# snayfach/MicrobeCensus

Hardware: AMD Instinct MI355X
Metric: reads/sec searched vs marker DB + AGS abs-error, 150 bp @ 1/2/4/8 GPU (higher is better)
Workload: dtype u8/int32

## Files before the change

### include/mcensus.h

```cpp
#ifndef MCENSUS_H
#define MCENSUS_H
#include <stdint.h>
#ifdef __cplusplus
extern "C" {
#endif

typedef struct mc_handle mc_handle;

typedef struct mc_row {
    int32_t query, subject;
    double ident;
    int32_t alnlen, mismatch, gapopen, qstart, qend, sstart, send;
    double loge, bits;
    int32_t score, nmatch;
} mc_row;

typedef struct mc_best_hit {
    int32_t read, family, aln, target_len;
    double bits;
} mc_best_hit;

typedef struct mc_stats {
    int64_t reads, seed_tasks, gap_tasks, hsps, rows, reads_with_rows, classified;
    int64_t bucket_lookups, key_probes;
// ... 34 lines not shown
int mc_search_classes(mc_handle *h, const uint8_t *rows, int64_t nreads, int32_t stride, int64_t first_read_id);
int64_t mc_result_best_classes(mc_handle *h, const uint8_t **cls);
int mc_result_class_reads(mc_handle *h, int64_t *out );
int64_t mc_debug_classes_prologue(mc_handle *h, const uint8_t *rows, int64_t nreads, int32_t stride, uint32_t *perm, uint32_t *start, int64_t *word0,
                                  uint8_t *sorted, int64_t sorted_cap, float *ms);

int mc_upload(mc_handle *h, const uint8_t *reads, int64_t nreads);
int mc_attach(mc_handle *h, const void *device_reads, int64_t nreads);
int mc_run(mc_handle *h, int64_t first_read_id);
int mc_run_range(mc_handle *h, int64_t first, int64_t count, int64_t first_read_id);

int mc_range_begin(mc_handle *h, int64_t first, int64_t count, int64_t first_read_id);
int mc_range_end(mc_handle *h);
int mc_ranges_in_flight(const mc_handle *h);
int64_t mc_ranges_translated_ahead(const mc_handle *h);

int64_t mc_debug_stage(mc_handle *h, int what, void *dst, int64_t cap_bytes, int32_t *record_bytes);
void mc_debug_live(int64_t out[4]);

int mc_set_counting(mc_handle *h, int on);

int64_t mc_result_rows(mc_handle *h, const mc_row **rows);
int64_t mc_result_best_hits(mc_handle *h, const mc_best_hit **hits);
int mc_result_stats(mc_handle *h, mc_stats *out);

int mc_write_m8(mc_handle *h, const char *path, int append);
int mc_write_m8_named(mc_handle *h, const char *path, int append, const char *const *query_names, int64_t n_names, int64_t first_read_id);

int mc_grid_classify(mc_handle *h, const double *aln_covs, int32_t n_cov, const int32_t *max_pids, int32_t n_pid, const double *min_scores, int32_t n_score,
                     int64_t *count_hits, int64_t *count_aln, double *count_cov);
// ... 111 lines not shown
```

### microbecensus_amd/_native.py

```python
import ctypes as C
import gzip
import json
import math
import os
import sys

import numpy as np

_HERE = os.path.dirname(os.path.abspath(__file__))
LIB_PATH = os.path.join(_HERE, "libmcensus_hip.so")
DATA_DIR = os.path.join(_HERE, "data")


class McRow(C.Structure):
    _fields_ = [("query", C.c_int32), ("subject", C.c_int32), ("ident", C.c_double), ("alnlen", C.c_int32),
                ("mismatch", C.c_int32), ("gapopen", C.c_int32), ("qstart", C.c_int32), ("qend", C.c_int32),
                ("sstart", C.c_int32), ("send", C.c_int32), ("loge", C.c_double), ("bits", C.c_double),
                ("score", C.c_int32), ("nmatch", C.c_int32)]


class McBestHit(C.Structure):
    _fields_ = [("read", C.c_int32), ("family", C.c_int32), ("aln", C.c_int32), ("target_len", C.c_int32),
                ("bits", C.c_double)]

# ... 66 lines not shown
    lib.mc_set_run.argtypes = [C.c_void_p, C.c_int32, C.c_double, C.POINTER(C.c_double), C.POINTER(C.c_double), C.POINTER(C.c_int32), C.POINTER(C.c_int32)]
    lib.mc_search.argtypes = [C.c_void_p, C.c_void_p, C.c_int64, C.c_int64]
    lib.mc_search_varlen.argtypes = [C.c_void_p, C.c_void_p, C.c_void_p, C.c_int64, C.c_int64]
    lib.mc_upload.argtypes = [C.c_void_p, C.c_void_p, C.c_int64]
    lib.mc_run.argtypes = [C.c_void_p, C.c_int64]
    lib.mc_attach.argtypes = [C.c_void_p, C.c_void_p, C.c_int64]
    lib.mc_run_range.argtypes = [C.c_void_p, C.c_int64, C.c_int64, C.c_int64]
    lib.mc_set_counting.argtypes = [C.c_void_p, C.c_int]
    lib.mc_debug_stage.restype = C.c_int64
    lib.mc_debug_stage.argtypes = [C.c_void_p, C.c_int, C.c_void_p, C.c_int64, C.POINTER(C.c_int32)]
    lib.mc_range_begin.argtypes = [C.c_void_p, C.c_int64, C.c_int64, C.c_int64]
    lib.mc_range_end.argtypes = [C.c_void_p]
    lib.mc_ranges_in_flight.argtypes = [C.c_void_p]
    lib.mc_ranges_translated_ahead.restype = C.c_int64
    lib.mc_ranges_translated_ahead.argtypes = [C.c_void_p]
    lib.mc_result_rows.restype = C.c_int64
    lib.mc_result_rows.argtypes = [C.c_void_p, C.POINTER(C.POINTER(McRow))]
    lib.mc_result_best_hits.restype = C.c_int64
    lib.mc_result_best_hits.argtypes = [C.c_void_p, C.POINTER(C.POINTER(McBestHit))]
    lib.mc_result_stats.argtypes = [C.c_void_p, C.POINTER(McStats)]
    lib.mc_write_m8.argtypes = [C.c_void_p, C.c_char_p, C.c_int]
    lib.mc_write_m8_named.argtypes = [C.c_void_p, C.c_char_p, C.c_int, C.POINTER(C.c_char_p), C.c_int64, C.c_int64]
    lib.mc_reader_last_error.restype = C.c_char_p
    lib.mc_set_host_threads.restype = None
    lib.mc_set_host_threads.argtypes = [C.c_int32]
    lib.mc_reader_open.restype = C.c_void_p
    lib.mc_reader_open.argtypes = [C.POINTER(C.c_char_p), C.c_int32, C.c_int32, C.c_int64, C.c_int32, C.c_int32, C.c_double, C.c_double, C.c_double, C.c_int32, C.c_char_p]
    lib.mc_reader_open_range.restype = C.c_void_p
    lib.mc_reader_open_range.argtypes = [C.c_char_p, C.c_int64, C.c_int64, C.c_int32, C.c_int64, C.c_int32, C.c_int32, C.c_double, C.c_double, C.c_double]
    lib.mc_reader_run.restype = C.c_int64
# ... 95 lines not shown
    lib.mc_coverage_depth.argtypes = [C.c_void_p, C.c_void_p, C.c_int64]
    lib.mc_coverage_ms.restype = C.c_float
    lib.mc_coverage_ms.argtypes = [C.c_void_p]
    lib.mc_set_ties.argtypes = [C.c_void_p, C.c_int, C.c_void_p, C.c_int32]
    lib.mc_ties_read.argtypes = [C.c_void_p, C.c_void_p, C.c_void_p, C.c_void_p, C.c_void_p, C.POINTER(C.c_int64), C.POINTER(C.c_int64)]
    lib.mc_ties_coverage_read.argtypes = [C.c_void_p, C.c_void_p, C.c_void_p, C.c_void_p]
    lib.mc_ties_ms.restype = C.c_float
    lib.mc_ties_ms.argtypes = [C.c_void_p]
    lib.mc_debug_live.restype = None
    lib.mc_debug_live.argtypes = [C.POINTER(C.c_int64)]
    _lib = lib
    return lib


EXPORTED_SYMBOLS = ["mc_last_error", "mc_device_count", "mc_open", "mc_close", "mc_set_index_cache", "mc_index_cache_check", "mc_open_rapdb", "mc_marker_count", "mc_marker_name", "mc_set_families", "mc_rapdb_verify", "mc_rapdb_write", "mc_index_view", "mc_set_run", "mc_search", "mc_search_varlen",
                    "mc_upload", "mc_attach", "mc_run", "mc_run_range", "mc_set_counting", "mc_debug_stage", "mc_range_begin", "mc_range_end", "mc_ranges_in_flight", "mc_ranges_translated_ahead", "mc_result_rows", "mc_result_best_hits", "mc_result_stats", "mc_write_m8", "mc_write_m8_named",
                    "mc_reader_last_error", "mc_set_host_threads", "mc_reader_open", "mc_reader_open_range", "mc_reader_open_bz2_part", "mc_bz2_blocks", "mc_gz_chunks", "mc_reader_open_gz_part", "mc_reader_gz_provide", "mc_reader_gz_end_state", "mc_reader_gz_finish", "mc_reader_run", "mc_reader_reads", "mc_reader_get_stats", "mc_reader_times", "mc_reader_describe", "mc_dupset_open", "mc_dupset_close", "mc_dupset_walk", "mc_reader_take", "mc_reader_close", "mc_reader_trim", "mc_count_bases", "mc_quality_offset",
                    "mc_reader_start", "mc_reader_fetch", "mc_reader_join", "mc_reader_read_len", "mc_reader_nreads", "mc_search_files", "mc_search_files_multi", "mc_set_keep_rows", "mc_set_best_hits_only", "mc_grid_classify", "mc_bootstrap", "mc_bootstrap_ms",
                    "mc_fit_weights", "mc_weights_mue", "mc_fit_weights_ms",
                    "mc_genome_open", "mc_genome_close", "mc_genome_set_library", "mc_simulate", "mc_train_library", "mc_train_times",
                    "mc_genome_set_read_lengths", "mc_simulate_varlen", "mc_train_library_bases",
                    "mc_community_open", "mc_community_close", "mc_community_set_library", "mc_community_simulate", "mc_community_library", "mc_community_member_reads",
                    "mc_community_times",
                    "mc_set_run_classes", "mc_search_classes", "mc_result_best_classes", "mc_result_class_reads", "mc_debug_classes_prologue", "mc_reader_open_classes", "mc_reader_stride",
                    "mc_set_abundance", "mc_abundance_reset", "mc_abundance_read", "mc_abundance_ms",
                    "mc_set_coverage", "mc_coverage_read", "mc_coverage_depth", "mc_coverage_ms",
                    "mc_set_ties", "mc_ties_read", "mc_ties_coverage_read", "mc_ties_ms", "mc_debug_live"]


class DupSet:

# ... 652 lines not shown
    def set_counting(self, on):
        self._check(self.lib.mc_set_counting(self.h, 1 if on else 0), "mc_set_counting")

    def range_begin(self, first, count, first_read_id=0):
        self._check(self.lib.mc_range_begin(self.h, first, count, first_read_id), "mc_range_begin")

    def range_end(self):
        self._check(self.lib.mc_range_end(self.h), "mc_range_end")

    def ranges_in_flight(self):
        return self.lib.mc_ranges_in_flight(self.h)

    def ranges_translated_ahead(self):
        return int(self.lib.mc_ranges_translated_ahead(self.h))

    def run_range(self, first, count, first_read_id=0):
        self._check(self.lib.mc_run_range(self.h, first, count, first_read_id), "mc_run_range")

    def debug_stage(self, what):
        rec = C.c_int32(0)
        n = self.lib.mc_debug_stage(self.h, what, None, 0, C.byref(rec))
        if n < 0:
            raise RuntimeError("mc_debug_stage failed: %s" % self.lib.mc_last_error().decode())
        buf = np.zeros(n, np.uint8)
        if n and self.lib.mc_debug_stage(self.h, what, buf.ctypes.data_as(C.c_void_p), n, C.byref(rec)) != n:
            raise RuntimeError("mc_debug_stage failed: %s" % self.lib.mc_last_error().decode())
        return buf.reshape(-1, rec.value) if rec.value else buf

    def gap_counts(self):
        v = self.debug_stage(4).reshape(-1).view("<u4")
# ... 142 lines not shown
```

### microbecensus_amd/csrc/mc_ahead.h

```cpp
#pragma once
#include <stdint.h>
#include <algorithm>

struct McAheadKey { uint64_t reads_gen; int64_t first, count; int32_t read_len, FP; uint64_t tables_gen; };
struct McAhead { McAheadKey key = {0, 0, 0, 0, 0, 0}; bool live = false; };

inline int64_t mc_ahead_predict(int64_t first, int64_t count, int64_t nreads, int64_t *next_first)
{
    *next_first = 0;
    if (first < 0 || count <= 0 || first > nreads - count) return 0;
    const int64_t at = first + count;
    const int64_t n = std::min(count, nreads - at);
    if (n <= 0) return 0;
    *next_first = at;
    return n;
}

inline void mc_ahead_offer(McAhead &a, const McAheadKey &k) { a.key = k; a.live = true; }

inline void mc_ahead_drop(McAhead &a) { a.live = false; }

inline int64_t mc_ahead_take(McAhead &a, const McAheadKey &want)
{
    const bool was = a.live;
    a.live = false;
    const McAheadKey &k = a.key;
    if (!was || want.count <= 0 || k.count <= 0 || k.reads_gen != want.reads_gen || k.first != want.first || k.read_len != want.read_len || k.FP != want.FP || k.tables_gen != want.tables_gen) return 0;
    return std::min(k.count, want.count);
}
```

### microbecensus_amd/csrc/mc_hip.hip

```cpp
#include "mc_hip_common.h"
#include "k_translate_seg.h"
#include "k_enumerate.h"
#include "k_eval_seeds.h"
#include "k_gapped.h"
#include "k_order.h"
#include "k_finish.h"
#include "k_grid.h"
#include "k_simulate.h"
#include "k_community.h"
#include "k_varlen.h"
#include "k_classes.h"
#include "k_bootstrap.h"
#include "k_wfit.h"
#include "mc_pieces.h"
#include "mc_ahead.h"
#include "mc_owned.h"
#include "mc_abund.h"

#include <map>

struct McCtx {
    McStream stream; hipStream_t side = nullptr, side2 = nullptr;
    McEvent ev[8], ev_fork, ev_join, ev_join2;
    int64_t cap_reads = 0; int pool_len = 0;
    int ts_staged = -1;
    uint32_t cap_tasks = 0, cap_gaps = 0, cap_hsps = 0, cap_rows = 0;
    McDev<uint8_t> d_frames_base; uint8_t *d_frames = nullptr;
    McDev<unsigned long long> d_stats;
    McDev<McSeedTask> d_tasks; McDev<McGapTask> d_gaps; McDev<McHsp> d_hsps, d_v, d_tmp;
    McDev<uint64_t> d_k64, d_hkeys, d_hplace, d_places; McDev<uint32_t> d_idx, d_idxo, d_heads, d_scan, d_gsz, d_nv, d_ghist;
    McDev<uint32_t> d_counters;
    McDev<McRow> d_rows; McDev<uint32_t> d_nrow, d_rowoff; McDev<McBestHit> d_best, d_bestof; McDev<uint8_t> d_low, d_cand;
    McDev<McGapCell> d_gws_full; McDev<uint32_t> d_retry, d_retry2; int gap_threads_full = 0;
    McDev<unsigned long long> d_gtab; uint32_t gtab_slots = 0; McDev<uint32_t> d_gleader; McDev<McFlankOut> d_fout;
    McPin<uint32_t> h_c; McPin<unsigned long long> h_stats; McPin<McBestHit> h_best; size_t h_best_cap = 0;
    const uint8_t *reads = nullptr; int64_t n = 0, first_read_id = 0, first = 0;
    int ahead_from = -1;
    bool own_a0 = true;
    uint32_t ntasks = 0, ngaps = 0, gpad = 0, nh = 0, nh_all = 0, nheads = 0, nrows = 0, nbest = 0, nsegs = 0;
    bool busy = false;
};

struct mc_handle {
    McHostIndex H;
    std::vector<int32_t> fam;
    int nfam = 0, device = 0;
    McDev<uint8_t> d_res_base; uint8_t *d_res = nullptr; McDev<uint32_t> d_off, d_bstart, d_post; McDev<unsigned long long> d_post8; McDev<uint16_t> d_keys; McDev<int32_t> d_fam;
    McDev<McTables> d_T; McDev<McClassPars> d_P;
    McTables hT; McClassPars hP;
    int read_len = 0, FP = 0; bool run_set = false;
    McDev<uint32_t> d_bitmap;
    McDev<McBucketRec> d_rec;
// ... 5 lines not shown
    bool best_only = false;
    bool rows_stay = false;
    float train_ms[3] = {0, 0, 0};
    float comm_ms[2] = {0, 0};
    int64_t train_bases = 0;
    float boot_ms = 0;
    float wfit_ms = 0;
    McAbundance ab;
    McPin<uint8_t> stage_pin[2]; McDev<uint8_t> stage_dev[2]; size_t stage_bytes = 0; McStream copy_stream;
    int64_t nreads = 0, cap_own = 0;
    McDev<uint8_t> d_reads;
    const uint8_t *reads_dev = nullptr;
    McCtx ctx;
    McStream ahead_stream; McEvent ahead_ev[2][2]; int ahead_p = 0; bool ahead_wait = false;
    McAhead ahead; uint64_t reads_gen = 0, tables_gen = 0; int64_t ahead_used = 0;
    McPin<mc_row> pin_slot[2]; size_t pin_slot_cap[2] = {0, 0}; int pin_cur = 0;
    McStream side, side2;
    McStream rows_stream; McEvent ev_rows; bool rows_pending = false, rows_ever = false;
    std::vector<mc_row> all_rows, split_rows;
    const mc_row *res_rows = nullptr; int64_t n_res_rows = 0;
    std::vector<mc_best_hit> best; mc_stats stats;
    McCtx *best_from = nullptr; uint32_t best_count = 0;
    std::map<int, McTables> vl_tables; double vl_thr = 0;
    McClasses cls = {}; bool cls_set = false, cls_results = false; std::vector<McClassPars> cls_pars;
    std::vector<uint8_t> best_cls; int64_t cls_reads[MC_CL_BINS] = {};
};

static void ahead_drop(mc_handle *h)
{
    if (h->ahead_wait) { (void)hipStreamSynchronize(h->ahead_stream); h->ahead_wait = false; }
// ... 56 lines not shown
static int open_impl(mc_handle *h, const int32_t *marker_family, int32_t nfam, int32_t device)
{
    int ndev = 0;
    double t0 = mc_now();
    if (hipGetDeviceCount(&ndev) != hipSuccess || ndev <= 0) { g_err = "no HIP device available: libmcensus_hip has no CPU fallback"; return -1; }
    if (device < 0 || device >= ndev) { g_err = "device index out of range"; return -1; }
    if (nfam > 32) { g_err = "at most 32 gene families are supported"; return -1; }
    const int nseq = h->H.nseq;
    if (nseq > 32767) { g_err = "more than 32767 markers: the HSP sort key (read<<43 | subject<<28 | hit order) holds 15 bits of subject index"; return -1; }
    for (int s = 0; s < nseq; s++) if ((int)(h->H.off[s + 1] - h->H.off[s]) > MC_GAP_W - 8) { g_err = "marker longer than the gapped-extension workspace"; return -1; }
    if (marker_family) h->fam.assign(marker_family, marker_family + nseq); else h->fam.assign((size_t)nseq, 0);
    h->nfam = nfam; h->device = device;
    HIPCK(hipSetDevice(device));
    HIPCK(hipFree(nullptr));
    MC_OT("  HIP runtime, device", t0);
    if (h->side.create() || h->side2.create()) return -1;
    {
        McCtx &c = h->ctx;
        if (c.stream.create()) return -1;
        c.side = h->side; c.side2 = h->side2;
        for (auto &e : c.ev) if (e.create()) return -1;
        if (c.ev_fork.create(false) || c.ev_join.create(false) || c.ev_join2.create(false)) return -1;
        if (c.d_counters.alloc(C_N) || c.d_stats.alloc(S_N) || c.d_ghist.alloc((size_t)MC_GS_BINS)) return -1;
        if (c.h_c.alloc(C_N) || c.h_stats.alloc(S_N)) return -1;
    }
    if (h->rows_stream.create() || h->ev_rows.create(false)) return -1;
    if (h->ahead_stream.create()) return -1;
    for (auto &pair : h->ahead_ev) for (auto &e : pair) if (e.create()) return -1;
    const McHostIndex &H = h->H;
    if (H.res.size() >= MC_TASK_ABS_LIMIT) { g_err = "marker database too large: more than 16 M residues (MC_TASK_W3)"; return -1; }
    if (h->d_res_base.alloc(H.res.size() + 128) || h->d_off.alloc(H.off.size()) || h->d_bstart.alloc(H.bstart.size()) || h->d_post.alloc(H.post.size() + 1) || h->d_post8.alloc((H.post.size() + 1) * MC_POST_WORDS) ||
        h->d_keys.alloc(H.keys.size()) || h->d_fam.alloc((size_t)nseq) || h->d_T.alloc(1) || h->d_P.alloc(1)) return -1;
    HIPCK(hipMemset(h->d_res_base, MC_INV, H.res.size() + 128));
    h->d_res = h->d_res_base + 64;
    h->ab.bind(nseq, (size_t)H.nres, h->d_off);
    if (h->d_bitmap.alloc(H.bitmap.size()) || h->d_filt.alloc(H.filt.size()) || h->d_wild.alloc(H.wild.size()) || h->d_pair.alloc(H.pair.size()) || h->d_rt.alloc(H.rt.size())) return -1;
    if (!H.rec.empty() && h->d_rec.alloc(H.rec.size())) return -1;
    {
        McUploader up;
        if (up.init() || up.put(h->d_res, H.res.data(), H.res.size()) || up.put(h->d_off, H.off.data(), H.off.size() * 4) || up.put(h->d_bstart, H.bstart.data(), H.bstart.size() * 4) ||
            up.put(h->d_post, H.post.data(), H.post.size() * 4) || up.put(h->d_keys, H.keys.data(), H.keys.size() * 2) || up.put(h->d_fam, h->fam.data(), (size_t)nseq * 4) ||
            up.put(h->d_bitmap, H.bitmap.data(), H.bitmap.size() * 4) || up.put(h->d_pair, H.pair.data(), H.pair.size() * 4) || up.put(h->d_wild, H.wild.data(), H.wild.size() * 4) ||
// ... 176 lines not shown
{
    if (nreads <= c.cap_reads && h->read_len <= c.pool_len) return 0;
    if (h->best_from == &c) best_materialize(h);
    ahead_drop(h);
    double t0 = mc_now();
    int64_t cap = nreads;
    if (cap > (1 << 21) - 1) { g_err = "batch larger than 2097151 reads"; return -1; }
    const int64_t L = h->read_len;
    c.cap_reads = 0;
    c.cap_tasks = (uint32_t)std::min<int64_t>(cap * (L + 32) + (1 << 20) + (int64_t)256 * 32 * MC_EN_BLK, 0x7fffffff);
    const int64_t ev_pad = (int64_t)256 * 8 * (MC_EV_BS / 64) * MC_EV_BLK;
    c.cap_gaps = (uint32_t)std::min<int64_t>(cap * (L / 8 + 8) + (1 << 18) + ev_pad, (1 << 27) - 2);
    c.cap_hsps = (uint32_t)std::min<int64_t>(cap * (L / 3 + 8) + (1 << 20) + ev_pad, 0x7fffffff);
    c.cap_rows = (uint32_t)std::min<int64_t>(cap * 16 + (1 << 20), 0x7fffffff);
    c.gap_threads_full = 16 * 1024;
    if (c.d_frames_base.alloc((size_t)cap * 6 * h->FP + 128) || c.d_tasks.alloc(c.cap_tasks) ||
        c.d_gaps.alloc(c.cap_gaps) || c.d_hsps.alloc(c.cap_hsps) || c.d_v.alloc(c.cap_hsps) ||
        c.d_tmp.alloc((size_t)c.cap_hsps * 2) || c.d_k64.alloc(c.cap_hsps) || c.d_hkeys.alloc(c.cap_hsps) || c.d_hplace.alloc(c.cap_hsps) || c.d_places.alloc(c.cap_hsps) || c.d_idx.alloc(c.cap_hsps) ||
        c.d_idxo.alloc(c.cap_hsps) || c.d_heads.alloc((size_t)cap + 2) || c.d_scan.alloc((size_t)4100) || c.d_gsz.alloc(c.cap_hsps) || c.d_nv.alloc((size_t)cap + 1) || c.d_rows.alloc(c.cap_rows) ||
        c.d_low.alloc((size_t)cap + 64) || c.d_cand.alloc((size_t)cap + 64) || c.d_nrow.alloc((size_t)cap + 1) || c.d_rowoff.alloc((size_t)cap + 1) || c.d_best.alloc((size_t)cap + 1) || c.d_bestof.alloc((size_t)cap + 1) ||
        c.d_gws_full.alloc((size_t)c.gap_threads_full * MC_GAP_W) || c.d_retry.alloc((size_t)c.cap_gaps * 2 + (size_t)cap + 1) || c.d_retry2.alloc((size_t)c.cap_gaps * 2) || c.d_gleader.alloc((size_t)c.cap_gaps) ||
        c.d_fout.alloc((size_t)c.cap_gaps * 2))
        return -1;
    c.d_frames = c.d_frames_base + 64;
    HIPCK(hipMemsetAsync(c.d_frames_base, MC_INV, 64, c.stream));
    if (c.h_best.alloc((size_t)cap + 1)) return -1;
    c.h_best_cap = (size_t)cap + 1;
    c.cap_reads = cap; c.pool_len = (int)L;
    HIPCK(hipStreamSynchronize(c.stream));
    MC_OT("ensure_capacity (pools)", t0);
    return 0;
}

static int reads_reserve(mc_handle *h, int64_t nreads)
{
    const int64_t need = nreads * (int64_t)h->read_len + 16;
    if (need > h->cap_own) { reads_change(h); if (h->d_reads.alloc((size_t)need)) return -1; h->cap_own = need; }
    return 0;
}

// ... 70 lines not shown
            fprintf(stderr, "fh-worst read: %llu stacked HSPs, %.3f Mcycles:", w[0] & 0xFFFFF, (double)(w[0] >> 20) / 1e6);
            for (int k = 0; k < 8; k++) fprintf(stderr, " %s %.3f", nm[k], (double)w[1 + k] / 1e6);
            fprintf(stderr, "\n");
            unsigned long long z12[12] = {0, 0, 0, 0, 0, 0, 0, 0, 0, 0, 0, 0};
            HIPCK(hipMemcpyToSymbol(HIP_SYMBOL(g_fh_worst), z12, sizeof z12));
        }
        unsigned long long z[8] = {0, 0, 0, 0, 0, 0, 0, 0};
        HIPCK(hipMemcpyToSymbol(HIP_SYMBOL(g_fh_acc), z, sizeof z)); HIPCK(hipMemcpyToSymbol(HIP_SYMBOL(g_fh_cnt), z, sizeof z));
    }
    return 0;
}
#else
static int exp_timing_dump(mc_handle *, McCtx &, char) { return 0; }
#endif

static int stage_a0(mc_handle *h, McCtx &c, hipStream_t st, const uint8_t *reads, int64_t at, int64_t n, hipEvent_t e0, hipEvent_t e1)
{
    const int L = h->read_len, FP = h->FP;
    uint8_t *frames = c.d_frames + at * 6 * FP;
    HIPCK(hipEventRecord(e0, st));
    const size_t lds_rest = (size_t)MC_TS_NLNF(FP) * 8 + (size_t)MC_TS_THREADS * MC_TS_STRIDE(FP);
    const size_t lds_staged = (size_t)MC_TS_STAGE(L) + lds_rest, lds_direct = (size_t)MC_TS_STAGE(0) + lds_rest;
    static const int ts_force = getenv("MC_TS_STAGED") ? atoi(getenv("MC_TS_STAGED")) : -1;
    const size_t cu_lds = 160 * 1024 - 1024;
    const bool staged = ts_force >= 0 ? ts_force != 0 : cu_lds / lds_staged >= cu_lds / lds_direct;
    const size_t lds = staged ? lds_staged : lds_direct;
    c.ts_staged = staged ? 1 : 0;
    const unsigned ts_blocks = (unsigned)((n + MC_TS_READS - 1) / MC_TS_READS);
    if (staged) {
        if (lds > 48 * 1024) HIPCK(hipFuncSetAttribute((const void *)k_translate_seg<true>, hipFuncAttributeMaxDynamicSharedMemorySize, (int)lds));
        k_translate_seg<true><<<dim3(ts_blocks), dim3(MC_TS_THREADS), lds, st>>>(h->d_T, reads, L, n, frames, FP, h->d_segtab);
    } else {
        if (lds > 48 * 1024) HIPCK(hipFuncSetAttribute((const void *)k_translate_seg<false>, hipFuncAttributeMaxDynamicSharedMemorySize, (int)lds));
        k_translate_seg<false><<<dim3(ts_blocks), dim3(MC_TS_THREADS), lds, st>>>(h->d_T, reads, L, n, frames, FP, h->d_segtab);
// ... 3 lines not shown
}

static int stage_a(mc_handle *h, McCtx &c, int64_t covered)
{
    const int64_t n = c.n;
    const int L = h->read_len, FP = h->FP;
    hipStream_t st = c.stream;
    McIndex X = dev_index(h);
    c.ntasks = c.ngaps = c.gpad = c.nh = c.nheads = c.nrows = c.nbest = c.nsegs = 0;
    HIPCK(hipMemsetAsync(c.d_counters, 0, sizeof(uint32_t) * C_N, st));
    HIPCK(hipMemsetAsync(c.d_stats, 0, sizeof(unsigned long long) * S_N, st));
    if (h->best_only) HIPCK(hipMemsetAsync(c.d_cand, 0, (size_t)n, st));
    HIPCK(hipMemsetAsync(c.d_low, 0, (size_t)n, st));
    c.own_a0 = covered < n;
    if (!c.own_a0) HIPCK(hipEventRecord(c.ev[1], st));
    else if (stage_a0(h, c, st, c.reads + covered * L, covered, n - covered, c.ev[0], c.ev[1])) return -1;
    if (exp_timing_dump(h, c, 'a')) return -1;
    const int64_t threads = n * 6;
    if (h->fast_enum) {
        const bool enq = !h->count_traffic;
        const size_t per_wave = enq ? MC_ENQ_WAVE_LDS(FP, L) : sizeof(McEnWave) + MC_EN_WAVE_LDS(FP, L);
        int waves = 0, bpc = 1;
        {
            static const int shapes_q[][2] = {{8, 2}, {4, 4}, {16, 1}, {12, 1}, {4, 3}, {8, 1}, {4, 2}, {4, 1}};
            static const int shapes_c[][2] = {{12, 2}, {8, 3}, {4, 6}, {4, 5}, {16, 1}, {8, 2}, {4, 4}, {12, 1}, {4, 3}, {8, 1}, {4, 2}, {4, 1}};
            if (enq) { for (const auto &sh : shapes_q) if (!waves && (size_t)sh[1] * (64 + sh[0] * per_wave) <= 160 * 1024) { waves = sh[0]; bpc = sh[1]; } }
            else for (const auto &sh : shapes_c) if (!waves && (size_t)sh[1] * (64 + sh[0] * per_wave) <= 160 * 1024) { waves = sh[0]; bpc = sh[1]; }
        }
        if (!waves) { g_err = "reads too long for the seed kernel's LDS layout"; return -1; }
        const size_t lds2 = 64 + waves * per_wave;
#define MC_LAUNCH_EN(KERNEL, WV)                                                                                                                   \
// ... 193 lines not shown
    McResults R(true, &h->split_rows);
    R.tot.range_splits = 1;
    int64_t off = 0, step = std::max<int64_t>(1, count / 2);
    while (off < count) {
        const int64_t nb = std::min<int64_t>(step, count - off);
        rc = run_range_once(h, first + off, nb, first_read_id + off);
        if (rc == -2 && nb > 1) { step = std::max<int64_t>(1, nb / 2); R.tot.range_splits++; continue; }
        if (rc) return rc;
        R.take(h);
        off += nb;
    }
    h->res_rows = R.rows.data(); h->n_res_rows = (int64_t)R.rows.size(); h->best.swap(R.best); h->best_from = nullptr; h->stats = R.tot;
    return 0;
}

static int range_begin(mc_handle *h, McCtx &c, int64_t first, int64_t count, int64_t first_read_id)
{
    if (ensure_capacity(h, c, count)) return -1;
    c.reads = h->reads_dev + first * h->read_len; c.n = count; c.first_read_id = first_read_id; c.first = first;
    const int64_t covered = mc_ahead_take(h->ahead, ahead_key(h, first, count));
    if (h->ahead_wait) { HIPCK(hipStreamWaitEvent(c.stream, h->ahead_ev[h->ahead_p][1], 0)); h->ahead_wait = false; }
    c.ahead_from = covered ? h->ahead_p : -1;
    if (covered) { h->ahead_used++; h->ahead_p ^= 1; }
    const int rc = stage_a(h, c, covered);
    if (rc) { (void)hipStreamSynchronize(c.stream); return rc; }
    c.busy = true;
    return 0;
}

static int ahead_issue(mc_handle *h, McCtx &c, int64_t first, int64_t count)
{
    if (count <= 0 || count > c.cap_reads || h->read_len > c.pool_len || first < 0 || first + count > h->nreads || !h->reads_dev) return 0;
    ahead_drop(h);
    HIPCK(hipStreamWaitEvent(h->ahead_stream, c.ev[4], 0));
    h->ahead_wait = true;
    if (stage_a0(h, c, h->ahead_stream, h->reads_dev + first * h->read_len, 0, count, h->ahead_ev[h->ahead_p][0], h->ahead_ev[h->ahead_p][1])) { ahead_drop(h); return -1; }
    mc_ahead_offer(h->ahead, ahead_key(h, first, count));
    return 0;
}

static void best_materialize(mc_handle *h)
{
    McCtx *c = h->best_from;
    if (!c) return;
    h->best_from = nullptr;
    const uint32_t nb = h->best_count;
    std::sort(c->h_best.get(), c->h_best + nb, [](const McBestHit &x, const McBestHit &y) { return x.read < y.read; });
    h->best.resize(nb);
    for (uint32_t i = 0; i < nb; i++) { const McBestHit &x = c->h_best[i]; mc_best_hit &o = h->best[i]; o.read = x.read; o.family = x.family; o.aln = x.aln; o.target_len = x.target_len; o.bits = x.bits; }
}

static int range_end(mc_handle *h, McCtx &c, int64_t next_first = 0, int64_t next_count = 0)
{
    c.busy = false;
    h->cls_results = false;
    memset(&h->stats, 0, sizeof h->stats);
    h->res_rows = nullptr; h->n_res_rows = 0; h->best.clear(); h->best_from = nullptr;
    h->stats.reads = c.n;
    int rc = stage_wait(c);
    if (rc == 0) rc = stage_b(h, c);
    if (rc == 0 && MC_AHEAD_ON) rc = ahead_issue(h, c, next_first, next_count);
    if (rc == 0 && (rc = stage_wait(c)) == 0 && (rc = stage_c(h, c)) == 0) rc = stage_d(h, c);
    if (rc == 0) rc = stage_wait(c);
    if (rc == 0 && c.h_c[C_OVERFLOW]) { g_err = "row buffer overflow"; rc = -2; }
    if (rc) { (void)hipStreamSynchronize(c.stream); ahead_drop(h); return rc; }
    h->pin_cur ^= 1;
    c.nrows = (c.nh && !h->best_only) ? c.h_c[C_ROWS] : 0u; c.nsegs = c.h_c[C_SEGS]; c.nbest = c.h_c[C_BEST];
    const bool abund = h->ab.active() && !h->best_only;
    if (abund && h->ab.launch(c.d_rows, std::min(c.nrows, c.cap_rows), c.stream)) return -1;
    if ((size_t)c.nrows > h->pin_slot_cap[h->pin_cur] && !rows_stay(h)) {
        (void)hipStreamSynchronize(h->rows_stream);
        const size_t want = (size_t)c.nrows + c.nrows / 4 + 1024;
        McPin<mc_row> nb, ob;
        if (nb.alloc(want)) { g_err = "out of pinned host memory for the rows"; return -1; }
        h->pin_slot[h->pin_cur] = std::move(nb); h->pin_slot_cap[h->pin_cur] = want;
        const int other = h->pin_cur ^ 1;
        if (h->pin_slot_cap[other] < want && ob.alloc(want) == 0) { h->pin_slot[other] = std::move(ob); h->pin_slot_cap[other] = want; }
    }
    rc = stage_e(h, c);
    if (rc) { (void)hipStreamSynchronize(c.stream); (void)hipStreamSynchronize(h->rows_stream); return rc; }
    if (c.nrows && !rows_stay(h)) { HIPCK(hipEventRecord(h->ev_rows, h->rows_stream)); h->rows_pending = true; h->rows_ever = true; }
    if ((rc = stage_wait(c)) != 0) return rc;
    if (abund) h->ab.range_done(c.n);
    h->res_rows = rows_stay(h) ? nullptr : (const mc_row *)h->pin_slot[h->pin_cur]; h->n_res_rows = rows_stay(h) ? 0 : (int64_t)c.nrows;
    h->best_from = &c; h->best_count = c.nbest;
#ifdef MC_EXP_TIMING
    { const char *nm[6] = {"staging/other", "append", "lookup", "push", "setup", "expand"}; for (int k = 0; k < 6; k++) fprintf(stderr, "timing %-14s %8.3f Mcycles/wave-avg  %10llu entries\n", nm[k], (double)c.h_stats[4 + k] / 4096.0 / 1e6, c.h_stats[10 + k]); }
#endif
    h->stats.bucket_lookups += (int64_t)c.h_stats[S_LOOKUPS]; h->stats.key_probes += (int64_t)c.h_stats[S_KEYPROBES]; h->stats.seed_tasks += (int64_t)c.h_stats[S_TASKS];
    h->stats.seed_exact_asks += (int64_t)c.h_stats[S_EXACT]; h->stats.seed_wild_asks += (int64_t)c.h_stats[S_WILD]; h->stats.seed_pair_asks += (int64_t)c.h_stats[S_PAIRS]; h->stats.seed_probes += (int64_t)c.h_stats[S_PROBES];
    h->stats.gap_tasks += c.ngaps - c.gpad; h->stats.hsps += c.nh_all; h->stats.rows += c.nrows; h->stats.reads_with_rows += c.nsegs;
    const float ms_tr = (c.own_a0 ? ev_ms(c.ev[0], c.ev[1]) : 0.0f) + (c.ahead_from >= 0 ? ev_ms(h->ahead_ev[c.ahead_from][0], h->ahead_ev[c.ahead_from][1]) : 0.0f);
    h->stats.ms_translate += ms_tr; h->stats.ms_seed += ev_ms(c.ev[1], c.ev[2]); h->stats.ms_eval += ev_ms(c.ev[2], c.ev[3]);
    h->stats.ms_gapped += ev_ms(c.ev[3], c.ev[4]); h->stats.ms_sort += ev_ms(c.ev[4], c.ev[5]); h->stats.ms_finish += ev_ms(c.ev[5], c.ev[6]); h->stats.ms_total += ms_tr + ev_ms(c.ev[1], c.ev[6]);
    h->stats.classified = (int64_t)c.nbest;
    return 0;
}

static int range_check(mc_handle *h, int64_t first, int64_t count)
{
    if (!h || !h->run_set) { g_err = "mc_set_run() must be called first"; return -1; }
    if (first < 0 || count < 0 || first + count > h->nreads) { g_err = "range outside the resident read set"; return -1; }
    if (count > (1 << 21) - 1) { g_err = "batch larger than 2097151 reads"; return -1; }
    HIPCK(hipSetDevice(h->device));
    return 0;
}

static int run_range_once(mc_handle *h, int64_t first, int64_t count, int64_t first_read_id)
{
    if (range_check(h, first, count)) return -1;
    if (count == 0) { memset(&h->stats, 0, sizeof h->stats); h->res_rows = nullptr; h->n_res_rows = 0; h->best.clear(); h->best_from = nullptr; return 0; }
    McCtx &c = h->ctx;
    const int rc = range_begin(h, c, first, count, first_read_id);
    if (rc) return rc;
    return range_end(h, c);
}

extern "C" int mc_range_begin(mc_handle *h, int64_t first, int64_t count, int64_t first_read_id)
{
    if (range_check(h, first, count)) return -1;
    if (count <= 0) { g_err = "mc_range_begin: an empty range"; return -1; }
    if (h->pipe_nout) { g_err = "mc_range_begin: a range is in flight already (mc_range_end first)"; return -1; }
    const int rc = range_begin(h, h->ctx, first, count, first_read_id);
    if (rc) return rc;
    h->pipe_nout = 1;
    return 0;
}

static int range_end_next(mc_handle *h, int64_t first, int64_t count, bool predict)
{
    if (predict) count = mc_ahead_predict(h->ctx.first, h->ctx.n, h->nreads, &first);
    return range_end(h, h->ctx, first, count);
}

extern "C" int64_t mc_ranges_translated_ahead(const mc_handle *h) { return h ? h->ahead_used : 0; }

extern "C" int mc_range_end(mc_handle *h)
{
    if (!h) { g_err = "null handle"; return -1; }
    if (h->pipe_nout == 0) { g_err = "mc_range_end: no range in flight"; return -1; }
    HIPCK(hipSetDevice(h->device));
    h->pipe_nout = 0;
    return range_end_next(h, 0, 0, true);
}

extern "C" int mc_ranges_in_flight(const mc_handle *h) { return h ? h->pipe_nout : 0; }

extern "C" int64_t mc_debug_stage(mc_handle *h, int what, void *dst, int64_t cap_bytes, int32_t *record_bytes)
{
    if (!h || !h->run_set || what < 0 || what > 5) { g_err = "mc_debug_stage: bad argument"; return -1; }
    if (h->pipe_nout) { g_err = "mc_debug_stage: ranges are in flight"; return -1; }
    HIPCK(hipSetDevice(h->device));
    ahead_drop(h);
    const McCtx &c = h->ctx;
    if (what == 4) {
        if (!c.h_c) { g_err = "mc_debug_stage: no range has run"; return -1; }
        const uint32_t v[3] = {c.h_c[C_ITEMS], c.h_c[C_RETRY], c.h_c[C_RETRY2]};
        if (record_bytes) *record_bytes = (int32_t)sizeof(uint32_t);
// ... 79 lines not shown
            cv.notify_all();
            if (rc <= 0) return;
        }
    });
    h->all_rows.clear();
    if (h->keep_rows && expect_reads > 0) h->all_rows.reserve((size_t)expect_reads * 2 + 1024);
    McResults R(h->keep_rows, &h->all_rows);
    const uint8_t *saved_reads = h->reads_dev; const int64_t saved_n = h->nreads;
    bool pending = false;
    auto collect = [&]() { if (pending) { pending = false; R.take(h); } };
    auto release = [&](int k) { std::unique_lock<std::mutex> lk(mu); slot[k].state = 0; cv.notify_all(); };
    auto reads_at = [&](int k) { reads_change(h); h->reads_dev = slot[k].dev; h->nreads = slot[k].n; };
    auto end_batch = [&](int k, int next) -> int {
        if (next >= 0) reads_at(next);
        h->pipe_nout = 0;
        int r = range_end_next(h, 0, next >= 0 ? slot[next].n : 0, false);
        if (r == -2) { reads_at(k); r = mc_run_range(h, 0, slot[k].n, first_read_id + slot[k].first); if (next >= 0) reads_at(next); }
        if (r) return r;
        pending = true;
        release(k);
        return 0;
    };
    int rc = 0, flying = -1;
    for (int k = 0;; k ^= 1) {
        {
            bool ready;
            { std::unique_lock<std::mutex> lk(mu); ready = slot[k].state != 0; }
            if (!ready && flying >= 0) { if ((rc = end_batch(flying, -1)) != 0) break; flying = -1; collect(); }
        }
        { std::unique_lock<std::mutex> lk(mu); cv.wait(lk, [&] { return slot[k].state != 0; }); }
        if (slot[k].state == 2) { if (slot[k].rc < 0) { rc = (int)slot[k].rc; if (!up_err.empty()) g_err = up_err; } break; }
        if (flying >= 0) { if ((rc = end_batch(flying, k)) != 0) break; flying = -1; }
        else reads_at(k);
        if ((rc = mc_range_begin(h, 0, slot[k].n, first_read_id + slot[k].first)) != 0) break;
        flying = k;
        collect();
    }
    if (rc == 0 && flying >= 0) { rc = end_batch(flying, -1); flying = -1; }
    if (rc == 0) collect();
    if (h->pipe_nout) { h->pipe_nout = 0; (void)range_end(h, h->ctx); }
    ahead_drop(h);
    { std::unique_lock<std::mutex> lk(mu); abort_up = true; cv.notify_all(); }
    uploader.join();
    reads_change(h);
    h->reads_dev = saved_reads; h->nreads = saved_n;
    if (rc) return rc;
    h->res_rows = R.rows.data(); h->n_res_rows = (int64_t)R.rows.size(); h->best.swap(R.best); h->best_from = nullptr; h->stats = R.tot;
    return 0;
}
// ... 103 lines not shown
        if (e == hipSuccess && pars) e = hipMemcpy(h->d_P, &h->hP, sizeof(McClassPars), hipMemcpyHostToDevice);
        if (rc == 0 && e != hipSuccess) { g_err = std::string("restoring the run's tables: ") + hipGetErrorString(e); rc = -1; }
        return rc;
    }
};

template <class BlockOf> static int run_pieces(mc_handle *h, McLenBorrow &len, const std::vector<McPiece> &pieces, BlockOf block_of, const McClassPars *pars, McResults &R)
{
    auto same_bin = [](const McPiece &a, const McPiece &b) { return a.tag == b.tag && a.L == b.L && a.bin_first == b.bin_first && a.bin_n == b.bin_n; };
    auto begin = [&](const McPiece &q, const McPiece *before) -> int {
        if (!before || !same_bin(*before, q)) {
            if (len.use(q.L, pars ? pars + q.tag : nullptr)) return -1;
            reads_change(h);
            h->reads_dev = block_of(q); h->nreads = q.bin_n;
        }
        return mc_range_begin(h, q.first, q.n, q.bin_first + q.first);
    };
    int rc = pieces.empty() ? 0 : begin(pieces[0], nullptr);
    for (size_t j = 0; rc == 0 && j < pieces.size(); j++) {
        const McPiece &q = pieces[j];
        const McPiece *nx = j + 1 < pieces.size() ? &pieces[j + 1] : nullptr;
        const bool ahead = nx && same_bin(q, *nx);
        h->pipe_nout = 0;
        rc = range_end_next(h, ahead ? nx->first : 0, ahead ? nx->n : 0, false);
        if (rc == -2) rc = mc_run_range(h, q.first, q.n, q.bin_first + q.first);
        if (rc) break;
        if (nx && (rc = begin(*nx, &q)) != 0) break;
        R.take(h, q.tag);
    }
    if (h->pipe_nout) { h->pipe_nout = 0; (void)range_end(h, h->ctx); }
    ahead_drop(h);
    return rc;
}


static int vl_bucket(McDevBuf &B, hipStream_t st, const uint8_t *d_bases, const int64_t *d_off, int64_t nreads, int64_t total, uint8_t **d_sorted,
                     uint32_t **d_perm, std::vector<uint32_t> &start, std::vector<int64_t> &boff)
{
    const uint32_t ntiles = (uint32_t)((nreads + MC_VL_TILE - 1) / MC_VL_TILE);
// ... 919 lines not shown
}

extern "C" int mc_simulate(mc_genome *g, int32_t read_len, int64_t first, int64_t n, uint64_t seed, uint64_t library_id, uint8_t *dst_host)
{
    if (!g || first < 0 || n < 0 || (n > 0 && !dst_host)) { g_err = "mc_simulate: bad argument"; return -1; }
    if (simulate_begin(g, read_len)) return -1;
    if (n == 0) return 0;
    return simulate_to_host(g, read_len, first, n, sim_key(seed, library_id), dst_host, "mc_simulate");
}

static int train_range(mc_handle *h, int64_t first, int64_t count, int64_t first_read_id, const McGridPars &G, unsigned long long *d_bins, size_t nbins,
                       hipEvent_t e0, hipEvent_t e1, mc_stats &tot)
{
    if (count <= 0) return 0;
    McCtx &c = h->ctx;
    int rc = range_begin(h, c, first, count, first_read_id);
    if (rc == 0) rc = range_end(h, c);
    if (rc == -2 && count > 1) {
        tot.range_splits++;
        const int64_t a = count / 2;
        if ((rc = train_range(h, first, a, first_read_id, G, d_bins, nbins, e0, e1, tot)) != 0) return rc;
        return train_range(h, first + a, count - a, first_read_id + a, G, d_bins, nbins, e0, e1, tot);
    }
    if (rc) return rc;
    stats_add(tot, h->stats);
    const int64_t nrows = (int64_t)c.nrows;
    HIPCK(hipEventRecord(e0, c.stream));
    if (nrows) k_grid_classify<<<dim3((unsigned)((nrows + 127) / 128)), dim3(128), 0, c.stream>>>(G, dev_index(h), h->d_fam, c.d_rows, nrows, d_bins, d_bins + nbins, (double *)(d_bins + 2 * nbins));
    HIPCK(hipEventRecord(e1, c.stream));
    HIPCK(hipEventSynchronize(e1));
    h->train_ms[2] += ev_ms(e0, e1);
// ... 209 lines not shown
```

Before: 66.25 million.

## Double-buffer translated frames so look-ahead translation overlaps the current range

Adds a second translated-frames buffer and alternates between them, so the next range's translation can write into the spare buffer while the current range still reads its own. For the public range_begin API, the look-ahead translation is now issued right after the current translation finishes, no longer after the gapped stage, which lets it overlap seeding and the later stages. The stream wait on the ahead event is only recorded when the event has not completed yet, and wait time is counted as translate time. This costs a second frames allocation and adds buffer-swap bookkeeping that must stay consistent with how ahead results are taken.

```diff
diff --git a/include/mcensus.h b/include/mcensus.h
--- a/include/mcensus.h
+++ b/include/mcensus.h
@@ -72,6 +72,7 @@
 int mc_range_end(mc_handle *h);
 int mc_ranges_in_flight(const mc_handle *h);
 int64_t mc_ranges_translated_ahead(const mc_handle *h);
+float mc_ahead_kernel_ms(const mc_handle *h);
 
 int64_t mc_debug_stage(mc_handle *h, int what, void *dst, int64_t cap_bytes, int32_t *record_bytes);
 void mc_debug_live(int64_t out[4]);
diff --git a/microbecensus_amd/_native.py b/microbecensus_amd/_native.py
--- a/microbecensus_amd/_native.py
+++ b/microbecensus_amd/_native.py
@@ -104,6 +104,8 @@
     lib.mc_ranges_in_flight.argtypes = [C.c_void_p]
     lib.mc_ranges_translated_ahead.restype = C.c_int64
     lib.mc_ranges_translated_ahead.argtypes = [C.c_void_p]
+    lib.mc_ahead_kernel_ms.restype = C.c_float
+    lib.mc_ahead_kernel_ms.argtypes = [C.c_void_p]
     lib.mc_result_rows.restype = C.c_int64
     lib.mc_result_rows.argtypes = [C.c_void_p, C.POINTER(C.POINTER(McRow))]
     lib.mc_result_best_hits.restype = C.c_int64
@@ -229,7 +231,7 @@
 
 
 EXPORTED_SYMBOLS = ["mc_last_error", "mc_device_count", "mc_open", "mc_close", "mc_set_index_cache", "mc_index_cache_check", "mc_open_rapdb", "mc_marker_count", "mc_marker_name", "mc_set_families", "mc_rapdb_verify", "mc_rapdb_write", "mc_index_view", "mc_set_run", "mc_search", "mc_search_varlen",
-                    "mc_upload", "mc_attach", "mc_run", "mc_run_range", "mc_set_counting", "mc_debug_stage", "mc_range_begin", "mc_range_end", "mc_ranges_in_flight", "mc_ranges_translated_ahead", "mc_result_rows", "mc_result_best_hits", "mc_result_stats", "mc_write_m8", "mc_write_m8_named",
+                    "mc_upload", "mc_attach", "mc_run", "mc_run_range", "mc_set_counting", "mc_debug_stage", "mc_range_begin", "mc_range_end", "mc_ranges_in_flight", "mc_ranges_translated_ahead", "mc_ahead_kernel_ms", "mc_result_rows", "mc_result_best_hits", "mc_result_stats", "mc_write_m8", "mc_write_m8_named",
                     "mc_reader_last_error", "mc_set_host_threads", "mc_reader_open", "mc_reader_open_range", "mc_reader_open_bz2_part", "mc_bz2_blocks", "mc_gz_chunks", "mc_reader_open_gz_part", "mc_reader_gz_provide", "mc_reader_gz_end_state", "mc_reader_gz_finish", "mc_reader_run", "mc_reader_reads", "mc_reader_get_stats", "mc_reader_times", "mc_reader_describe", "mc_dupset_open", "mc_dupset_close", "mc_dupset_walk", "mc_reader_take", "mc_reader_close", "mc_reader_trim", "mc_count_bases", "mc_quality_offset",
                     "mc_reader_start", "mc_reader_fetch", "mc_reader_join", "mc_reader_read_len", "mc_reader_nreads", "mc_search_files", "mc_search_files_multi", "mc_set_keep_rows", "mc_set_best_hits_only", "mc_grid_classify", "mc_bootstrap", "mc_bootstrap_ms",
                     "mc_fit_weights", "mc_weights_mue", "mc_fit_weights_ms",
@@ -912,6 +914,9 @@
     def ranges_translated_ahead(self):
         return int(self.lib.mc_ranges_translated_ahead(self.h))
 
+    def ahead_kernel_ms(self):
+        return float(self.lib.mc_ahead_kernel_ms(self.h))
+
     def run_range(self, first, count, first_read_id=0):
         self._check(self.lib.mc_run_range(self.h, first, count, first_read_id), "mc_run_range")
 
diff --git a/microbecensus_amd/csrc/mc_ahead.h b/microbecensus_amd/csrc/mc_ahead.h
--- a/microbecensus_amd/csrc/mc_ahead.h
+++ b/microbecensus_amd/csrc/mc_ahead.h
@@ -3,7 +3,7 @@
 #include <algorithm>
 
 struct McAheadKey { uint64_t reads_gen; int64_t first, count; int32_t read_len, FP; uint64_t tables_gen; };
-struct McAhead { McAheadKey key = {0, 0, 0, 0, 0, 0}; bool live = false; };
+struct McAhead { McAheadKey key = {0, 0, 0, 0, 0, 0}; bool live = false; int cur = 0, buf = 1; };
 
 inline int64_t mc_ahead_predict(int64_t first, int64_t count, int64_t nreads, int64_t *next_first)
 {
@@ -16,7 +16,9 @@
     return n;
 }
 
-inline void mc_ahead_offer(McAhead &a, const McAheadKey &k) { a.key = k; a.live = true; }
+inline int mc_ahead_target(const McAhead &a) { return a.cur ^ 1; }
+
+inline void mc_ahead_offer(McAhead &a, const McAheadKey &k) { a.key = k; a.buf = mc_ahead_target(a); a.live = true; }
 
 inline void mc_ahead_drop(McAhead &a) { a.live = false; }
 
@@ -26,5 +28,6 @@
     a.live = false;
     const McAheadKey &k = a.key;
     if (!was || want.count <= 0 || k.count <= 0 || k.reads_gen != want.reads_gen || k.first != want.first || k.read_len != want.read_len || k.FP != want.FP || k.tables_gen != want.tables_gen) return 0;
+    a.cur = a.buf;
     return std::min(k.count, want.count);
 }
diff --git a/microbecensus_amd/csrc/mc_hip.hip b/microbecensus_amd/csrc/mc_hip.hip
--- a/microbecensus_amd/csrc/mc_hip.hip
+++ b/microbecensus_amd/csrc/mc_hip.hip
@@ -22,10 +22,13 @@
 struct McCtx {
     McStream stream; hipStream_t side = nullptr, side2 = nullptr;
     McEvent ev[8], ev_fork, ev_join, ev_join2;
+    McEvent ev_wait[2]; bool waited = false;
     int64_t cap_reads = 0; int pool_len = 0;
     int ts_staged = -1;
     uint32_t cap_tasks = 0, cap_gaps = 0, cap_hsps = 0, cap_rows = 0;
-    McDev<uint8_t> d_frames_base; uint8_t *d_frames = nullptr;
+    McDev<uint8_t> d_frames_base[2]; uint8_t *d_frames = nullptr;
+    uint8_t *frames_of(int b) const { return d_frames_base[b] + 64; }
+    void frames_use(int b) { d_frames = frames_of(b); }
     McDev<unsigned long long> d_stats;
     McDev<McSeedTask> d_tasks; McDev<McGapTask> d_gaps; McDev<McHsp> d_hsps, d_v, d_tmp;
     McDev<uint64_t> d_k64, d_hkeys, d_hplace, d_places; McDev<uint32_t> d_idx, d_idxo, d_heads, d_scan, d_gsz, d_nv, d_ghist;
@@ -36,6 +39,7 @@
     McPin<uint32_t> h_c; McPin<unsigned long long> h_stats; McPin<McBestHit> h_best; size_t h_best_cap = 0;
     const uint8_t *reads = nullptr; int64_t n = 0, first_read_id = 0, first = 0;
     int ahead_from = -1;
+    bool predicts = false;
     bool own_a0 = true;
     uint32_t ntasks = 0, ngaps = 0, gpad = 0, nh = 0, nh_all = 0, nheads = 0, nrows = 0, nbest = 0, nsegs = 0;
     bool busy = false;
@@ -71,6 +75,7 @@
     McCtx ctx;
     McStream ahead_stream; McEvent ahead_ev[2][2]; int ahead_p = 0; bool ahead_wait = false;
     McAhead ahead; uint64_t reads_gen = 0, tables_gen = 0; int64_t ahead_used = 0;
+    float ahead_ms = 0;
     McPin<mc_row> pin_slot[2]; size_t pin_slot_cap[2] = {0, 0}; int pin_cur = 0;
     McStream side, side2;
     McStream rows_stream; McEvent ev_rows; bool rows_pending = false, rows_ever = false;
@@ -157,18 +162,18 @@
     HIPCK(hipSetDevice(device));
     HIPCK(hipFree(nullptr));
     MC_OT("  HIP runtime, device", t0);
+    if (h->ctx.stream.create() || h->ahead_stream.create()) return -1;
     if (h->side.create() || h->side2.create()) return -1;
     {
         McCtx &c = h->ctx;
-        if (c.stream.create()) return -1;
         c.side = h->side; c.side2 = h->side2;
         for (auto &e : c.ev) if (e.create()) return -1;
         if (c.ev_fork.create(false) || c.ev_join.create(false) || c.ev_join2.create(false)) return -1;
+        for (auto &e : c.ev_wait) if (e.create()) return -1;
         if (c.d_counters.alloc(C_N) || c.d_stats.alloc(S_N) || c.d_ghist.alloc((size_t)MC_GS_BINS)) return -1;
         if (c.h_c.alloc(C_N) || c.h_stats.alloc(S_N)) return -1;
     }
     if (h->rows_stream.create() || h->ev_rows.create(false)) return -1;
-    if (h->ahead_stream.create()) return -1;
     for (auto &pair : h->ahead_ev) for (auto &e : pair) if (e.create()) return -1;
     const McHostIndex &H = h->H;
     if (H.res.size() >= MC_TASK_ABS_LIMIT) { g_err = "marker database too large: more than 16 M residues (MC_TASK_W3)"; return -1; }
@@ -375,7 +380,7 @@
     c.cap_hsps = (uint32_t)std::min<int64_t>(cap * (L / 3 + 8) + (1 << 20) + ev_pad, 0x7fffffff);
     c.cap_rows = (uint32_t)std::min<int64_t>(cap * 16 + (1 << 20), 0x7fffffff);
     c.gap_threads_full = 16 * 1024;
-    if (c.d_frames_base.alloc((size_t)cap * 6 * h->FP + 128) || c.d_tasks.alloc(c.cap_tasks) ||
+    if (c.d_frames_base[0].alloc((size_t)cap * 6 * h->FP + 128) || c.d_frames_base[1].alloc((size_t)cap * 6 * h->FP + 128) || c.d_tasks.alloc(c.cap_tasks) ||
         c.d_gaps.alloc(c.cap_gaps) || c.d_hsps.alloc(c.cap_hsps) || c.d_v.alloc(c.cap_hsps) ||
         c.d_tmp.alloc((size_t)c.cap_hsps * 2) || c.d_k64.alloc(c.cap_hsps) || c.d_hkeys.alloc(c.cap_hsps) || c.d_hplace.alloc(c.cap_hsps) || c.d_places.alloc(c.cap_hsps) || c.d_idx.alloc(c.cap_hsps) ||
         c.d_idxo.alloc(c.cap_hsps) || c.d_heads.alloc((size_t)cap + 2) || c.d_scan.alloc((size_t)4100) || c.d_gsz.alloc(c.cap_hsps) || c.d_nv.alloc((size_t)cap + 1) || c.d_rows.alloc(c.cap_rows) ||
@@ -383,8 +388,8 @@
         c.d_gws_full.alloc((size_t)c.gap_threads_full * MC_GAP_W) || c.d_retry.alloc((size_t)c.cap_gaps * 2 + (size_t)cap + 1) || c.d_retry2.alloc((size_t)c.cap_gaps * 2) || c.d_gleader.alloc((size_t)c.cap_gaps) ||
         c.d_fout.alloc((size_t)c.cap_gaps * 2))
         return -1;
-    c.d_frames = c.d_frames_base + 64;
-    HIPCK(hipMemsetAsync(c.d_frames_base, MC_INV, 64, c.stream));
+    c.frames_use(h->ahead.cur);
+    for (auto &b : c.d_frames_base) HIPCK(hipMemsetAsync(b, MC_INV, 64, c.stream));
     if (c.h_best.alloc((size_t)cap + 1)) return -1;
     c.h_best_cap = (size_t)cap + 1;
     c.cap_reads = cap; c.pool_len = (int)L;
@@ -485,10 +490,10 @@
 static int exp_timing_dump(mc_handle *, McCtx &, char) { return 0; }
 #endif
 
-static int stage_a0(mc_handle *h, McCtx &c, hipStream_t st, const uint8_t *reads, int64_t at, int64_t n, hipEvent_t e0, hipEvent_t e1)
+static int stage_a0(mc_handle *h, McCtx &c, hipStream_t st, const uint8_t *reads, uint8_t *into, int64_t at, int64_t n, hipEvent_t e0, hipEvent_t e1)
 {
     const int L = h->read_len, FP = h->FP;
-    uint8_t *frames = c.d_frames + at * 6 * FP;
+    uint8_t *frames = into + at * 6 * FP;
     HIPCK(hipEventRecord(e0, st));
     const size_t lds_rest = (size_t)MC_TS_NLNF(FP) * 8 + (size_t)MC_TS_THREADS * MC_TS_STRIDE(FP);
     const size_t lds_staged = (size_t)MC_TS_STAGE(L) + lds_rest, lds_direct = (size_t)MC_TS_STAGE(0) + lds_rest;
@@ -522,7 +527,7 @@
     HIPCK(hipMemsetAsync(c.d_low, 0, (size_t)n, st));
     c.own_a0 = covered < n;
     if (!c.own_a0) HIPCK(hipEventRecord(c.ev[1], st));
-    else if (stage_a0(h, c, st, c.reads + covered * L, covered, n - covered, c.ev[0], c.ev[1])) return -1;
+    else if (stage_a0(h, c, st, c.reads + covered * L, c.d_frames, covered, n - covered, c.ev[0], c.ev[1])) return -1;
     if (exp_timing_dump(h, c, 'a')) return -1;
     const int64_t threads = n * 6;
     if (h->fast_enum) {
@@ -746,27 +751,40 @@
     return 0;
 }
 
-static int range_begin(mc_handle *h, McCtx &c, int64_t first, int64_t count, int64_t first_read_id)
+static int ahead_issue(mc_handle *h, McCtx &c, int64_t first, int64_t count, hipEvent_t behind);
+static int range_begin(mc_handle *h, McCtx &c, int64_t first, int64_t count, int64_t first_read_id, bool predicts)
 {
     if (ensure_capacity(h, c, count)) return -1;
-    c.reads = h->reads_dev + first * h->read_len; c.n = count; c.first_read_id = first_read_id; c.first = first;
+    c.reads = h->reads_dev + first * h->read_len; c.n = count; c.first_read_id = first_read_id; c.first = first; c.predicts = predicts;
     const int64_t covered = mc_ahead_take(h->ahead, ahead_key(h, first, count));
-    if (h->ahead_wait) { HIPCK(hipStreamWaitEvent(c.stream, h->ahead_ev[h->ahead_p][1], 0)); h->ahead_wait = false; }
+    c.frames_use(h->ahead.cur);
+    c.waited = h->ahead_wait && hipEventQuery(h->ahead_ev[h->ahead_p][1]) != hipSuccess;
+    if (c.waited) {
+        HIPCK(hipEventRecord(c.ev_wait[0], c.stream));
+        HIPCK(hipStreamWaitEvent(c.stream, h->ahead_ev[h->ahead_p][1], 0));
+        HIPCK(hipEventRecord(c.ev_wait[1], c.stream));
+    }
+    h->ahead_wait = false;
     c.ahead_from = covered ? h->ahead_p : -1;
     if (covered) { h->ahead_used++; h->ahead_p ^= 1; }
-    const int rc = stage_a(h, c, covered);
+    int rc = stage_a(h, c, covered);
     if (rc) { (void)hipStreamSynchronize(c.stream); return rc; }
     c.busy = true;
-    return 0;
-}
-
-static int ahead_issue(mc_handle *h, McCtx &c, int64_t first, int64_t count)
+    if (predicts && MC_AHEAD_ON) {
+        int64_t next_first = 0;
+        const int64_t next_count = mc_ahead_predict(first, count, h->nreads, &next_first);
+        if ((rc = ahead_issue(h, c, next_first, next_count, c.ev[1])) != 0) { (void)hipStreamSynchronize(c.stream); c.busy = false; return rc; }
+    }
+    return 0;
+}
+
+static int ahead_issue(mc_handle *h, McCtx &c, int64_t first, int64_t count, hipEvent_t behind)
 {
     if (count <= 0 || count > c.cap_reads || h->read_len > c.pool_len || first < 0 || first + count > h->nreads || !h->reads_dev) return 0;
     ahead_drop(h);
-    HIPCK(hipStreamWaitEvent(h->ahead_stream, c.ev[4], 0));
+    if (behind) HIPCK(hipStreamWaitEvent(h->ahead_stream, behind, 0));
     h->ahead_wait = true;
-    if (stage_a0(h, c, h->ahead_stream, h->reads_dev + first * h->read_len, 0, count, h->ahead_ev[h->ahead_p][0], h->ahead_ev[h->ahead_p][1])) { ahead_drop(h); return -1; }
+    if (stage_a0(h, c, h->ahead_stream, h->reads_dev + first * h->read_len, c.frames_of(mc_ahead_target(h->ahead)), 0, count, h->ahead_ev[h->ahead_p][0], h->ahead_ev[h->ahead_p][1])) { ahead_drop(h); return -1; }
     mc_ahead_offer(h->ahead, ahead_key(h, first, count));
     return 0;
 }
@@ -791,7 +809,7 @@
     h->stats.reads = c.n;
     int rc = stage_wait(c);
     if (rc == 0) rc = stage_b(h, c);
-    if (rc == 0 && MC_AHEAD_ON) rc = ahead_issue(h, c, next_first, next_count);
+    if (rc == 0 && MC_AHEAD_ON && !c.predicts) rc = ahead_issue(h, c, next_first, next_count, c.ev[4]);
     if (rc == 0 && (rc = stage_wait(c)) == 0 && (rc = stage_c(h, c)) == 0) rc = stage_d(h, c);
     if (rc == 0) rc = stage_wait(c);
     if (rc == 0 && c.h_c[C_OVERFLOW]) { g_err = "row buffer overflow"; rc = -2; }
@@ -822,7 +840,8 @@
     h->stats.bucket_lookups += (int64_t)c.h_stats[S_LOOKUPS]; h->stats.key_probes += (int64_t)c.h_stats[S_KEYPROBES]; h->stats.seed_tasks += (int64_t)c.h_stats[S_TASKS];
     h->stats.seed_exact_asks += (int64_t)c.h_stats[S_EXACT]; h->stats.seed_wild_asks += (int64_t)c.h_stats[S_WILD]; h->stats.seed_pair_asks += (int64_t)c.h_stats[S_PAIRS]; h->stats.seed_probes += (int64_t)c.h_stats[S_PROBES];
     h->stats.gap_tasks += c.ngaps - c.gpad; h->stats.hsps += c.nh_all; h->stats.rows += c.nrows; h->stats.reads_with_rows += c.nsegs;
-    const float ms_tr = (c.own_a0 ? ev_ms(c.ev[0], c.ev[1]) : 0.0f) + (c.ahead_from >= 0 ? ev_ms(h->ahead_ev[c.ahead_from][0], h->ahead_ev[c.ahead_from][1]) : 0.0f);
+    const float ms_tr = (c.own_a0 ? ev_ms(c.ev[0], c.ev[1]) : 0.0f) + (c.waited ? ev_ms(c.ev_wait[0], c.ev_wait[1]) : 0.0f);
+    h->ahead_ms = c.ahead_from >= 0 ? ev_ms(h->ahead_ev[c.ahead_from][0], h->ahead_ev[c.ahead_from][1]) : 0.0f;
     h->stats.ms_translate += ms_tr; h->stats.ms_seed += ev_ms(c.ev[1], c.ev[2]); h->stats.ms_eval += ev_ms(c.ev[2], c.ev[3]);
     h->stats.ms_gapped += ev_ms(c.ev[3], c.ev[4]); h->stats.ms_sort += ev_ms(c.ev[4], c.ev[5]); h->stats.ms_finish += ev_ms(c.ev[5], c.ev[6]); h->stats.ms_total += ms_tr + ev_ms(c.ev[1], c.ev[6]);
     h->stats.classified = (int64_t)c.nbest;
@@ -843,29 +862,27 @@
     if (range_check(h, first, count)) return -1;
     if (count == 0) { memset(&h->stats, 0, sizeof h->stats); h->res_rows = nullptr; h->n_res_rows = 0; h->best.clear(); h->best_from = nullptr; return 0; }
     McCtx &c = h->ctx;
-    const int rc = range_begin(h, c, first, count, first_read_id);
+    const int rc = range_begin(h, c, first, count, first_read_id, false);
     if (rc) return rc;
     return range_end(h, c);
 }
 
-extern "C" int mc_range_begin(mc_handle *h, int64_t first, int64_t count, int64_t first_read_id)
+static int range_begin_checked(mc_handle *h, int64_t first, int64_t count, int64_t first_read_id, bool predicts)
 {
     if (range_check(h, first, count)) return -1;
     if (count <= 0) { g_err = "mc_range_begin: an empty range"; return -1; }
     if (h->pipe_nout) { g_err = "mc_range_begin: a range is in flight already (mc_range_end first)"; return -1; }
-    const int rc = range_begin(h, h->ctx, first, count, first_read_id);
+    const int rc = range_begin(h, h->ctx, first, count, first_read_id, predicts);
     if (rc) return rc;
     h->pipe_nout = 1;
     return 0;
 }
-
-static int range_end_next(mc_handle *h, int64_t first, int64_t count, bool predict)
-{
-    if (predict) count = mc_ahead_predict(h->ctx.first, h->ctx.n, h->nreads, &first);
-    return range_end(h, h->ctx, first, count);
-}
+extern "C" int mc_range_begin(mc_handle *h, int64_t first, int64_t count, int64_t first_read_id) { return range_begin_checked(h, first, count, first_read_id, true); }
+
+static int range_end_next(mc_handle *h, int64_t first, int64_t count) { return range_end(h, h->ctx, first, count); }
 
 extern "C" int64_t mc_ranges_translated_ahead(const mc_handle *h) { return h ? h->ahead_used : 0; }
+extern "C" float mc_ahead_kernel_ms(const mc_handle *h) { return h ? h->ahead_ms : 0.0f; }
 
 extern "C" int mc_range_end(mc_handle *h)
 {
@@ -873,7 +890,7 @@
     if (h->pipe_nout == 0) { g_err = "mc_range_end: no range in flight"; return -1; }
     HIPCK(hipSetDevice(h->device));
     h->pipe_nout = 0;
-    return range_end_next(h, 0, 0, true);
+    return range_end(h, h->ctx);
 }
 
 extern "C" int mc_ranges_in_flight(const mc_handle *h) { return h ? h->pipe_nout : 0; }
@@ -983,7 +1000,7 @@
     auto end_batch = [&](int k, int next) -> int {
         if (next >= 0) reads_at(next);
         h->pipe_nout = 0;
-        int r = range_end_next(h, 0, next >= 0 ? slot[next].n : 0, false);
+        int r = range_end_next(h, 0, next >= 0 ? slot[next].n : 0);
         if (r == -2) { reads_at(k); r = mc_run_range(h, 0, slot[k].n, first_read_id + slot[k].first); if (next >= 0) reads_at(next); }
         if (r) return r;
         pending = true;
@@ -1001,7 +1018,7 @@
         if (slot[k].state == 2) { if (slot[k].rc < 0) { rc = (int)slot[k].rc; if (!up_err.empty()) g_err = up_err; } break; }
         if (flying >= 0) { if ((rc = end_batch(flying, k)) != 0) break; flying = -1; }
         else reads_at(k);
-        if ((rc = mc_range_begin(h, 0, slot[k].n, first_read_id + slot[k].first)) != 0) break;
+        if ((rc = range_begin_checked(h, 0, slot[k].n, first_read_id + slot[k].first, false)) != 0) break;
         flying = k;
         collect();
     }
@@ -1135,7 +1152,7 @@
             reads_change(h);
             h->reads_dev = block_of(q); h->nreads = q.bin_n;
         }
-        return mc_range_begin(h, q.first, q.n, q.bin_first + q.first);
+        return range_begin_checked(h, q.first, q.n, q.bin_first + q.first, false);
     };
     int rc = pieces.empty() ? 0 : begin(pieces[0], nullptr);
     for (size_t j = 0; rc == 0 && j < pieces.size(); j++) {
@@ -1143,7 +1160,7 @@
         const McPiece *nx = j + 1 < pieces.size() ? &pieces[j + 1] : nullptr;
         const bool ahead = nx && same_bin(q, *nx);
         h->pipe_nout = 0;
-        rc = range_end_next(h, ahead ? nx->first : 0, ahead ? nx->n : 0, false);
+        rc = range_end_next(h, ahead ? nx->first : 0, ahead ? nx->n : 0);
         if (rc == -2) rc = mc_run_range(h, q.first, q.n, q.bin_first + q.first);
         if (rc) break;
         if (nx && (rc = begin(*nx, &q)) != 0) break;
@@ -2093,7 +2110,7 @@
 {
     if (count <= 0) return 0;
     McCtx &c = h->ctx;
-    int rc = range_begin(h, c, first, count, first_read_id);
+    int rc = range_begin(h, c, first, count, first_read_id, false);
     if (rc == 0) rc = range_end(h, c);
     if (rc == -2 && count > 1) {
         tot.range_splits++;
```

New measurement: 69.66 million (median of 6 runs). +5.2%, better.
